# tiangexiang/OccNeRF

Hardware: AMD Instinct MI355X
Metric: rays/sec at 512x512x128spp, random-init ckpt (higher is better)
Workload: dtype f32; 1 GPU; BASELINE configs[1]: free-view frame, 512x512 image, 128 samples/ray, non-rigid motion on, seeded random-init checkpoint; synthetic SMPL-like body and camera; 183784 rays hit the body bbox (ray_mask); H2D of the ray batch and the prior and D2H of [R,5] inside the step; the frame's rays sharded over the ranks; samples whose motion-weight sum is exactly 0 are dropped after the warp (bit-identical pi; rays_per_frame=183784, samples_per_ray=128, skip_empty_samples=True, dedup_repeated_samples=False, knn_center_cache=True, warp_bone_culling=True, world_size_formed=1

## Files before the change

occnerf_amd/csrc/nonrigid16.hip:

```cpp
#include "common.h"

namespace occ {
namespace nr16 {

typedef float f32x4 __attribute__((ext_vector_type(4)));

constexpr int kW = 128, kOB = kW / 16;
constexpr int kCond = 69, kEmb = 36;
constexpr int kKS_E = 9, kKS_H = kW / 4, kKS_Skip = kKS_H + kKS_E;
constexpr int groups_of(int ks) { return (ks + 3) / 4; }
constexpr int kC_E = groups_of(kKS_E);
constexpr int kC_H = groups_of(kKS_H);
constexpr int kC_Skip = groups_of(kKS_Skip);
constexpr int kChunks = kC_E + 3 * kC_H + kC_Skip + kC_H;
constexpr int kWaves = 4, kFrags = 2;
constexpr int kRingSlots = 4, kTailChunks = kRingSlots;
constexpr int kChunkF4 = 512;

enum Kind { kL0 = 0, kHidden = 1, kSkip = 2 };

__host__ __device__ inline int e_feature(int t, int g) {
    const int A = t < 8 ? (t >> 1) * 4 + g : 16 + (g >> 1);
    const int is_cos = t < 8 ? (t & 1) : (g & 1);
    return (A / 3) * 6 + is_cos * 3 + A % 3;
}

__host__ __device__ inline int slot_feature(int kind, int t, int g) {
    const int cd = 16 * (t >> 2) + 4 * g + (t & 3);
    switch (kind) {
        case kL0: return t < kKS_E ? kCond + e_feature(t, g) : -1;
        case kHidden: return t < kKS_H ? cd : -1;
        case kSkip:
            if (t < kKS_H) return cd;
            return t < kKS_Skip ? kW + e_feature(t - kKS_H, g) : -1;
    }
    return -1;
}

struct Aux {
    static constexpr int kL0B = 0;
    static constexpr int kHB = 128;
    static constexpr int kSkipB = 512;
    static constexpr int kL5B = 640;
    static constexpr int kOutW = 768;
    static constexpr int kOutB = 1152;
    static constexpr int kTotal = 1156;
};

struct Stream {
    static constexpr int64_t kChunkFloats = kChunkF4 * 4;
    static constexpr int64_t kL0 = 0;
    static constexpr int64_t kH = kL0 + kC_E * kChunkFloats;
    static constexpr int64_t kSkipW = kH + 3 * kC_H * kChunkFloats;
    static constexpr int64_t kL5 = kSkipW + kC_Skip * kChunkFloats;
    static constexpr int64_t kTail = kL5 + kC_H * kChunkFloats;
    static constexpr int64_t kAux = kTail + kTailChunks * kChunkFloats;
    static constexpr int64_t kTotal = kAux + Aux::kTotal;
};
static_assert(Stream::kTail == (int64_t)kChunks * Stream::kChunkFloats, "chunk stream is contiguous");

__global__ void pack_layer_kernel(const float *__restrict__ W, const float *__restrict__ b, int kind, int in_dim,
                                  int ks, float *__restrict__ Wp, float *__restrict__ Bp) {
    const int total = groups_of(ks) * kOB * 64 * 4;
    for (int e = blockIdx.x * blockDim.x + threadIdx.x; e < total; e += gridDim.x * blockDim.x) {
        const int rr = e & 3, lane = (e >> 2) & 63, rest = e >> 8;
        const int ob = rest % kOB, G = rest / kOB;
        const int t = 4 * G + rr;
        const int col = t < ks ? slot_feature(kind, t, lane >> 4) : -1;
        Wp[e] = col >= 0 ? W[(size_t)(ob * 16 + (lane & 15)) * in_dim + col] : 0.0f;
    }
    if (Bp)
        for (int e = blockIdx.x * blockDim.x + threadIdx.x; e < kW; e += gridDim.x * blockDim.x) Bp[e] = b[e];
}

__global__ void pack_rows_kernel(const float *__restrict__ W, const float *__restrict__ b, float *__restrict__ Wp,
                                 float *__restrict__ Bp) {
    for (int e = blockIdx.x * blockDim.x + threadIdx.x; e < 3 * kW; e += gridDim.x * blockDim.x) Wp[e] = W[e];
    if (blockIdx.x == 0 && threadIdx.x < 4) Bp[threadIdx.x] = threadIdx.x < 3 ? b[threadIdx.x] : 0.0f;
}

__global__ void fold_bias_kernel(const float *__restrict__ W0, const float *__restrict__ b0,
                                 const float *__restrict__ cond, float *__restrict__ Bp) {
    const int row = threadIdx.x;
    if (row >= kW) return;
    float acc = b0[row];
    for (int k = 0; k < kCond; k++) acc = __fmaf_rn(W0[(size_t)row * (kCond + kEmb) + k], cond[k], acc);
    Bp[row] = acc;
}

struct Params {
    float hann[6];
};

#define NR16_MFMA(a, b, c) __builtin_amdgcn_mfma_f32_16x16x4f32((a), (b), (c), 0, 0, 0)

__global__ __launch_bounds__(kWaves * 64, 2) void nonrigid_lds_kernel(const float *xyz_in , int64_t N_max,
                                                                      const int32_t *__restrict__ rows,
                                                                      const int32_t *__restrict__ n_dev,
                                                                      const float *__restrict__ pk, Params prm,
                                                                      float *xyz_out) {
    const int64_t N = n_dev ? (int64_t)*n_dev : N_max;
    const int64_t ntiles = (N + 32 * kWaves - 1) / (32 * kWaves);
    if ((int64_t)blockIdx.x >= ntiles) return;
    __shared__ __attribute__((aligned(16))) f32x4 smem[kRingSlots * kChunkF4 + Aux::kTotal / 4];
    f32x4 *ring = smem;
    float *aux = reinterpret_cast<float *>(smem + kRingSlots * kChunkF4);

    const int lane = threadIdx.x & 63;
    const int wave = __builtin_amdgcn_readfirstlane(threadIdx.x >> 6);
    const int s = lane & 15, g = lane >> 4;

    for (int i = threadIdx.x; i < Aux::kTotal; i += kWaves * 64) aux[i] = pk[Stream::kAux + i];

    const f32x4 *stream = reinterpret_cast<const f32x4 *>(pk);
    const unsigned ring_lds = (unsigned)(size_t)(__attribute__((address_space(3))) f32x4 *)ring;
    auto issue1 = [&](int c, int cs, int f) {
        const int frag = wave * kFrags + f;
        unsigned keep;
        asm volatile("s_mov_b32 %0, m0\n\ts_mov_b32 m0, %3\n\ts_nop 0\n\tglobal_load_lds_dwordx4 %1, %2\n\t"
                     "s_mov_b32 m0, %0"
                     : "=&s"(keep)
                     : "v"(lane * 16), "s"(stream + (size_t)cs * kChunkF4 + frag * 64),
                       "s"(ring_lds + (unsigned)(((c & (kRingSlots - 1)) * kChunkF4 + frag * 64) * 16))
                     : "memory");
    };
    auto issue = [&](int c, int cs) {
#pragma unroll
        for (int f = 0; f < kFrags; f++) issue1(c, cs, f);
    };
    int c = 0;
    int ci = 4;
    issue(0, 0);
    issue(1, 1);
    issue(2, 2);

    const f32x4 *slot_;
#define NR16_ENTER()                                                   \
    asm volatile("s_waitcnt vmcnt(4) lgkmcnt(0)" ::: "memory");        \
    __builtin_amdgcn_s_barrier();                                      \
    slot_ = ring + (c & (kRingSlots - 1)) * kChunkF4;                  \
    c++;
#define NR16_READ_HALF(W, HALF)                                        \
    _Pragma("unroll") for (int ob_ = 0; ob_ < 4; ob_++) W[ob_] = slot_[((HALF) * 4 + ob_) * 64 + lane];

    f32x4 wA[4];
    NR16_ENTER()
    issue(3, 3);
    NR16_READ_HALF(wA, 0)

    for (int64_t tile = blockIdx.x; tile < ntiles; tile += gridDim.x) {
    const int64_t base = (tile * kWaves + wave) * 32;

    float p[2][3], e[2][12];
    int32_t r_cur[2];
#pragma unroll
    for (int T = 0; T < 2; T++) {
        const int64_t n = base + T * 16 + s;
        const int64_t nm = n < N ? n : N - 1;
        r_cur[T] = rows ? rows[nm] : (int32_t)nm;
#pragma unroll
        for (int c = 0; c < 3; c++) p[T][c] = xyz_in[(int64_t)r_cur[T] * 3 + c];
#pragma unroll
        for (int m = 0; m < 5; m++) {
            const int A = m < 4 ? m * 4 + g : 16 + (g >> 1);
            const int oct = A / 3, c = A - 3 * oct;
            const float pc = c == 0 ? p[T][0] : (c == 1 ? p[T][1] : p[T][2]);
            const float wgt = oct == 0 ? prm.hann[0] : oct == 1 ? prm.hann[1] : oct == 2 ? prm.hann[2]
                            : oct == 3 ? prm.hann[3] : oct == 4 ? prm.hann[4] : prm.hann[5];
            const float a = __fmul_rn(pc, (float)(1 << oct));
            float sa, ca;
#ifdef OCC_NR16_EXP_NO_SINCOS
            sa = a, ca = 1.0f - a;
#else
            sincosf(a, &sa, &ca);
#endif
            const float sv = __fmul_rn(wgt, sa), cv = __fmul_rn(wgt, ca);
            if (m < 4) {
                e[T][2 * m] = sv;
                e[T][2 * m + 1] = cv;
            } else {
                e[T][8] = (g & 1) ? cv : sv;
            }
        }
        e[T][9] = e[T][10] = e[T][11] = 0.0f;
    }
#define NR16_HALF(W, HH, CL, KS, BOP)                                                            \
    _Pragma("unroll") for (int rr_ = 0; rr_ < 4; rr_++) {                                        \
        const int t_ = (CL) * 4 + rr_;                                                           \
        if ((HH) == 1 && rr_ < kFrags) {                                                         \
            issue1(c + 2, ci, rr_);                                                              \
            if (rr_ == kFrags - 1) ci = ci + 1 == kChunks ? 0 : ci + 1;                          \
        }                                                                                        \
        if (t_ < (KS)) {                                                                         \
            _Pragma("unroll") for (int ob_ = 0; ob_ < 4; ob_++) {                                \
                _Pragma("unroll") for (int T_ = 0; T_ < 2; T_++)                                 \
                    acc[T_][(HH) * 4 + ob_] = NR16_MFMA(W[ob_][rr_], BOP(T_, t_), acc[T_][(HH) * 4 + ob_]); \
            }                                                                                    \
        }                                                                                        \
    }
#define NR16_LAYER(CHUNKS, KS, BOP)                                                              \
    _Pragma("unroll") for (int c_ = 0; c_ < (CHUNKS); c_++) {                                    \
        f32x4 wB_[4];                                                                            \
        NR16_READ_HALF(wB_, 1)                                                                   \
        NR16_HALF(wA, 0, c_, KS, BOP)                                                            \
        NR16_ENTER()                                                                             \
        NR16_READ_HALF(wA, 0)                                                                    \
        NR16_HALF(wB_, 1, c_, KS, BOP)                                                           \
    }
#define NR16_BIAS(OFF)                                                                           \
    _Pragma("unroll") for (int ob_ = 0; ob_ < kOB; ob_++) {                                      \
        const f32x4 b_ = reinterpret_cast<const f32x4 *>(aux + (OFF))[ob_ * 4 + g];              \
        acc[0][ob_] = b_;                                                                        \
        acc[1][ob_] = b_;                                                                        \
    }
#define NR16_RELU()                                                                              \
    _Pragma("unroll") for (int T_ = 0; T_ < 2; T_++) {                                           \
        _Pragma("unroll") for (int ob_ = 0; ob_ < kOB; ob_++) {                                  \
            _Pragma("unroll") for (int r_ = 0; r_ < 4; r_++) act[T_][ob_][r_] = fmaxf(acc[T_][ob_][r_], 0.0f); \
        }                                                                                        \
    }

    f32x4 acc[2][kOB], act[2][kOB];
#define BOP_E(T, t) e[T][t]
#define BOP_A(T, t) act[T][(t) >> 2][(t) & 3]
#define BOP_SKIP(T, t) ((t) < kKS_H ? act[T][((t) >> 2) & 7][(t) & 3] : e[T][((t) - kKS_H) < 0 ? 0 : ((t) - kKS_H)])

    NR16_BIAS(Aux::kL0B)
    NR16_LAYER(kC_E, kKS_E, BOP_E)
    NR16_RELU()
#pragma unroll 1
    for (int l = 0; l < 4; l++) {
        if (l == 3) {
            NR16_BIAS(Aux::kSkipB)
            NR16_LAYER(kC_Skip, kKS_Skip, BOP_SKIP)
            NR16_RELU()
        }
        NR16_BIAS(l < 3 ? Aux::kHB + l * 128 : Aux::kL5B)
        NR16_LAYER(kC_H, kKS_H, BOP_A)
        NR16_RELU()
    }
#pragma unroll
    for (int T = 0; T < 2; T++) {
        float off[3];
#pragma unroll
        for (int ch = 0; ch < 3; ch++) {
            const f32x4 *W4 = reinterpret_cast<const f32x4 *>(aux + Aux::kOutW + ch * kW);
            float sum = 0.0f;
#pragma unroll
            for (int ob = 0; ob < kOB; ob++) {
                const f32x4 w = W4[ob * 4 + g];
#pragma unroll
                for (int r = 0; r < 4; r++) sum = __fmaf_rn(w[r], act[T][ob][r], sum);
            }
            sum += __shfl_xor(sum, 16);
            off[ch] = sum + __shfl_xor(sum, 32) + aux[Aux::kOutB + ch];
        }
        const int64_t n = base + T * 16 + s;
        if (g == 0 && n < N) {
            const int64_t nd = r_cur[T];
#pragma unroll
            for (int ch = 0; ch < 3; ch++) xyz_out[nd * 3 + ch] = __fadd_rn(p[T][ch], off[ch]);
        }
    }
    }
    asm volatile("s_waitcnt vmcnt(0)" ::: "memory");
#undef BOP_E
#undef BOP_A
#undef BOP_SKIP
#undef NR16_ENTER
#undef NR16_READ_HALF
#undef NR16_HALF
#undef NR16_LAYER
#undef NR16_BIAS
#undef NR16_RELU
}

}

int64_t nr_lds_packed_floats() { return nr16::Stream::kTotal; }

int nr_lds_pack(const float *const *h_W, const float *const *h_b, float *packed, hipStream_t st) {
    using namespace nr16;
    OCC_REQUIRE(hipMemsetAsync(packed + Stream::kTail, 0, sizeof(float) * (Stream::kTotal - Stream::kTail), st) ==
                    hipSuccess,
                "nonrigid_pack: memset failed");
    float *aux = packed + Stream::kAux;
    auto layer = [&](int li, int kind, int in_dim, int ks, int64_t woff, int boff) {
        hipLaunchKernelGGL(nr16::pack_layer_kernel, dim3(64), dim3(256), 0, st, h_W[li], h_b[li], kind, in_dim, ks,
                           packed + woff, boff >= 0 ? aux + boff : (float *)nullptr);
    };
    layer(0, kL0, kCond + kEmb, kKS_E, Stream::kL0, -1);
    for (int l = 0; l < 3; l++)
        layer(1 + l, kHidden, kW, kKS_H, Stream::kH + l * kC_H * Stream::kChunkFloats, Aux::kHB + l * 128);
    layer(4, kSkip, kW + kEmb, kKS_Skip, Stream::kSkipW, Aux::kSkipB);
    layer(5, kHidden, kW, kKS_H, Stream::kL5, Aux::kL5B);
    hipLaunchKernelGGL(nr16::pack_rows_kernel, dim3(2), dim3(256), 0, st, h_W[6], h_b[6], aux + Aux::kOutW,
                       aux + Aux::kOutB);
    return check_launch("nonrigid_pack");
}

int nr_lds_launch(const float *xyz_in, int64_t N, const int32_t *rows, const int32_t *n_dev, const float *cond,
                  const float *h_hann, const float *W0, const float *b0, float *packed, float *xyz_out,
                  hipStream_t st) {
    using namespace nr16;
    hipLaunchKernelGGL(nr16::fold_bias_kernel, dim3(1), dim3(128), 0, st, W0, b0, cond,
                       packed + Stream::kAux + Aux::kL0B);
    Params prm;
    for (int i = 0; i < 6; i++) prm.hann[i] = h_hann[i];
    const int64_t per_block = 32 * kWaves;
    int64_t blocks = (N + per_block - 1) / per_block;
    if (blocks > 2 * (int64_t)kNumCU) blocks = 2 * (int64_t)kNumCU;
    hipLaunchKernelGGL(nr16::nonrigid_lds_kernel, dim3((unsigned)blocks), dim3(64 * kWaves), 0, st, xyz_in, N, rows,
                       n_dev, packed, prm, xyz_out);
    return check_launch("nonrigid");
}

}
```

Measured before the change: 1.211 million rays/s.

## Double weight chunk size in nonrigid MLP ring, halving barriers per layer

After: 1.215 million rays/s (median of 6 runs). No clear change (+0.3%).

```diff
diff --git a/occnerf_amd/csrc/nonrigid16.hip b/occnerf_amd/csrc/nonrigid16.hip
--- a/occnerf_amd/csrc/nonrigid16.hip
+++ b/occnerf_amd/csrc/nonrigid16.hip
@@ -9,13 +9,16 @@
 constexpr int kCond = 69, kEmb = 36;
 constexpr int kKS_E = 9, kKS_H = kW / 4, kKS_Skip = kKS_H + kKS_E;
 constexpr int groups_of(int ks) { return (ks + 3) / 4; }
-constexpr int kC_E = groups_of(kKS_E);
-constexpr int kC_H = groups_of(kKS_H);
-constexpr int kC_Skip = groups_of(kKS_Skip);
+constexpr int kGroupsPerChunk = 2;
+constexpr int chunks_of(int ks) { return (groups_of(ks) + kGroupsPerChunk - 1) / kGroupsPerChunk; }
+constexpr int kC_E = chunks_of(kKS_E);
+constexpr int kC_H = chunks_of(kKS_H);
+constexpr int kC_Skip = chunks_of(kKS_Skip);
 constexpr int kChunks = kC_E + 3 * kC_H + kC_Skip + kC_H;
-constexpr int kWaves = 4, kFrags = 2;
+constexpr int kWaves = 4, kFrags = 4;
 constexpr int kRingSlots = 4, kTailChunks = kRingSlots;
-constexpr int kChunkF4 = 512;
+constexpr int kChunkF4 = 1024;
+static_assert(kChunks % kRingSlots == 0, "the ring phase repeats every tile: stream chunk i always lives in slot i & 3");
 
 enum Kind { kL0 = 0, kHidden = 1, kSkip = 2 };
 
@@ -61,7 +64,7 @@
 
 __global__ void pack_layer_kernel(const float *__restrict__ W, const float *__restrict__ b, int kind, int in_dim,
                                   int ks, float *__restrict__ Wp, float *__restrict__ Bp) {
-    const int total = groups_of(ks) * kOB * 64 * 4;
+    const int total = chunks_of(ks) * kGroupsPerChunk * kOB * 64 * 4;
     for (int e = blockIdx.x * blockDim.x + threadIdx.x; e < total; e += gridDim.x * blockDim.x) {
         const int rr = e & 3, lane = (e >> 2) & 63, rest = e >> 8;
         const int ob = rest % kOB, G = rest / kOB;
@@ -103,6 +106,7 @@
     const int64_t ntiles = (N + 32 * kWaves - 1) / (32 * kWaves);
     if ((int64_t)blockIdx.x >= ntiles) return;
     __shared__ __attribute__((aligned(16))) f32x4 smem[kRingSlots * kChunkF4 + Aux::kTotal / 4];
+    static_assert(2 * sizeof(smem) <= 160 * 1024, "two workgroups per CU share 160 KiB of LDS");
     f32x4 *ring = smem;
     float *aux = reinterpret_cast<float *>(smem + kRingSlots * kChunkF4);
 
@@ -134,19 +138,23 @@
     issue(1, 1);
     issue(2, 2);
 
+    static_assert(kFrags == 4, "NR16_ENTER waits with vmcnt(8) = 2 chunks x 4 DMAs per wave");
     const f32x4 *slot_;
+#define NR16_FENCE() __builtin_amdgcn_sched_barrier(0);
 #define NR16_ENTER()                                                   \
-    asm volatile("s_waitcnt vmcnt(4) lgkmcnt(0)" ::: "memory");        \
+    asm volatile("s_waitcnt vmcnt(8) lgkmcnt(0)" ::: "memory");        \
     __builtin_amdgcn_s_barrier();                                      \
+    NR16_FENCE()                                                       \
     slot_ = ring + (c & (kRingSlots - 1)) * kChunkF4;                  \
     c++;
-#define NR16_READ_HALF(W, HALF)                                        \
-    _Pragma("unroll") for (int ob_ = 0; ob_ < 4; ob_++) W[ob_] = slot_[((HALF) * 4 + ob_) * 64 + lane];
-
-    f32x4 wA[4];
+#define NR16_READ_QUARTER(W, Q)                                        \
+    _Pragma("unroll") for (int ob_ = 0; ob_ < 4; ob_++) W[ob_] = slot_[((Q) * 4 + ob_) * 64 + lane]; \
+    NR16_FENCE()
+
+    f32x4 wA[4], wB[4];
     NR16_ENTER()
     issue(3, 3);
-    NR16_READ_HALF(wA, 0)
+    NR16_READ_QUARTER(wA, 0)
 
     for (int64_t tile = blockIdx.x; tile < ntiles; tile += gridDim.x) {
     const int64_t base = (tile * kWaves + wave) * 32;
@@ -184,28 +192,32 @@
         }
         e[T][9] = e[T][10] = e[T][11] = 0.0f;
     }
-#define NR16_HALF(W, HH, CL, KS, BOP)                                                            \
+#define NR16_QUARTER(W, Q, CL, KS, BOP)                                                          \
     _Pragma("unroll") for (int rr_ = 0; rr_ < 4; rr_++) {                                        \
-        const int t_ = (CL) * 4 + rr_;                                                           \
-        if ((HH) == 1 && rr_ < kFrags) {                                                         \
+        const int t_ = ((CL) * kGroupsPerChunk + ((Q) >> 1)) * 4 + rr_;                          \
+        if ((Q) == 3) {                                                                          \
             issue1(c + 2, ci, rr_);                                                              \
             if (rr_ == kFrags - 1) ci = ci + 1 == kChunks ? 0 : ci + 1;                          \
         }                                                                                        \
         if (t_ < (KS)) {                                                                         \
             _Pragma("unroll") for (int ob_ = 0; ob_ < 4; ob_++) {                                \
                 _Pragma("unroll") for (int T_ = 0; T_ < 2; T_++)                                 \
-                    acc[T_][(HH) * 4 + ob_] = NR16_MFMA(W[ob_][rr_], BOP(T_, t_), acc[T_][(HH) * 4 + ob_]); \
+                    acc[T_][((Q) & 1) * 4 + ob_] = NR16_MFMA(W[ob_][rr_], BOP(T_, t_), acc[T_][((Q) & 1) * 4 + ob_]); \
             }                                                                                    \
         }                                                                                        \
-    }
+    }                                                                                            \
+    NR16_FENCE()
 #define NR16_LAYER(CHUNKS, KS, BOP)                                                              \
     _Pragma("unroll") for (int c_ = 0; c_ < (CHUNKS); c_++) {                                    \
-        f32x4 wB_[4];                                                                            \
-        NR16_READ_HALF(wB_, 1)                                                                   \
-        NR16_HALF(wA, 0, c_, KS, BOP)                                                            \
+        NR16_READ_QUARTER(wB, 1)                                                                 \
+        NR16_QUARTER(wA, 0, c_, KS, BOP)                                                         \
+        NR16_READ_QUARTER(wA, 2)                                                                 \
+        NR16_QUARTER(wB, 1, c_, KS, BOP)                                                         \
+        NR16_READ_QUARTER(wB, 3)                                                                 \
+        NR16_QUARTER(wA, 2, c_, KS, BOP)                                                         \
         NR16_ENTER()                                                                             \
-        NR16_READ_HALF(wA, 0)                                                                    \
-        NR16_HALF(wB_, 1, c_, KS, BOP)                                                           \
+        NR16_READ_QUARTER(wA, 0)                                                                 \
+        NR16_QUARTER(wB, 3, c_, KS, BOP)                                                         \
     }
 #define NR16_BIAS(OFF)                                                                           \
     _Pragma("unroll") for (int ob_ = 0; ob_ < kOB; ob_++) {                                      \
@@ -268,8 +280,9 @@
 #undef BOP_A
 #undef BOP_SKIP
 #undef NR16_ENTER
-#undef NR16_READ_HALF
-#undef NR16_HALF
+#undef NR16_READ_QUARTER
+#undef NR16_QUARTER
+#undef NR16_FENCE
 #undef NR16_LAYER
 #undef NR16_BIAS
 #undef NR16_RELU
```
